# ishine/TargetDiarization

Measured on AMD Instinct MI355X. Metric: real-time factor (audio-sec/wall-sec) full infer() pipe, 16kHz mono, 1/2/4/8 GPU, higher is better.
Workload: dtype f32 (split-f16 x3: fp32-accurate products from three f16 MFMA passes, fp32 accumulate); 1 GPU; BASELINE configs[3]: 1800 s synthetic conversation (two alternating speakers, 20 % overlap) = 180 x 10 s windows: MossFormer2 (90 windows per launch) -> loudness swap -> ERes2NetV2 on every 10 s window of both streams + cosine vs a target embedding -> Paraformer (SANM encoder, CIF predictor, NAR decoder, argmax tokens + timestamps) on 30 s segments of both streams -> CT-Transformer punctuation of ; windows_per_launch=90

## Files before the change

### targetdiarization_amd/_lib.py

```python
from __future__ import annotations

import ctypes as C
import os

HERE = os.path.dirname(os.path.abspath(__file__))
LIB_PATH = os.path.join(HERE, "libtdx.so")


class TdxError(RuntimeError):
    pass


class Mf2Config(C.Structure):
    _fields_ = [("num_blocks", C.c_int32), ("channels", C.c_int32), ("kernel_size", C.c_int32),
                ("num_spks", C.c_int32), ("group_size", C.c_int32), ("reserved", C.c_int32 * 3)]


class MdxConfig(C.Structure):
    _fields_ = [("num_blocks", C.c_int32), ("l", C.c_int32), ("g", C.c_int32), ("k", C.c_int32), ("bn", C.c_int32),
                ("dim_f", C.c_int32), ("dim_t", C.c_int32), ("reserved", C.c_int32)]


class WhisperConfig(C.Structure):
    _fields_ = [("n_mels", C.c_int32), ("n_audio_ctx", C.c_int32), ("d_model", C.c_int32), ("enc_heads", C.c_int32),
# ... 179 lines not shown
                           "(hipcc --offload-arch=gfx950).  There is no CPU fallback.")
        import torch
        tl = os.path.join(os.path.dirname(torch.__file__), "lib", "libamdhip64.so")
        if os.path.exists(tl):
            C.CDLL(tl, mode=C.RTLD_GLOBAL)
        l = C.CDLL(LIB_PATH)
        for name, (res, args) in SIGNATURES.items():
            fn = getattr(l, name)
            fn.restype = res
            fn.argtypes = args
        _lib = l
    return _lib


_l = C.c_long


class GemmSeg(C.Structure):
    _fields_ = [("A", _vp), ("B", _vp), ("lda", _l), ("ldb", _l), ("strideA", _l), ("strideB", _l), ("strideA2", _l), ("strideB2", _l),
                ("K", _i), ("zdiv", _i), ("kchunk", _i), ("ktotal", _i)]


class H3Seg(C.Structure):
    _fields_ = [("A", _vp), ("B", _vp), ("sa", _vp), ("sb", _vp), ("lda", _l), ("ldb", _l),
                ("strideA", _l), ("strideB", _l), ("strideA2", _l), ("strideB2", _l),
                ("strideSA", _l), ("strideSB", _l), ("strideSA2", _l), ("strideSB2", _l),
                ("sa_mul", _i), ("sb_mul", _i), ("K", _i), ("zdiv", _i), ("kchunk", _i), ("ktotal", _i), ("segk", _i),
                ("strideSeg", _l), ("a_shift", _i), ("a_period", _i), ("a_zero", _vp)]


DIAG_SIGNATURES = {
    "tdx_diag_last_error": (C.c_char_p, []),
    "tdx_h3_gemm_ex": (_i, [_i] * 4 + [C.POINTER(H3Seg)] * 2 + [_i] * 12 + [_vp, _vp, _l, _l, _i, C.POINTER(_i), _vp]),
    "tdx_h3_plan": (_i, [_i] * 5 + [C.POINTER(_i)] * 2),
    "tdx_h3_tile_of_block": (_i, [C.POINTER(_i), _i, _i, _i] + [C.POINTER(_i)] * 3),
    "tdx_h3_split_rows_static": (_i, [_vp, _l, _vp, _l, _i, C.c_float, _vp]),
    "tdx_h3_split_rows_long": (_i, [_vp, _l, _vp, _vp, _l, _i, _vp]),
    "tdx_h3_split_kmajor_ex": (_i, [_vp, _l, _vp, _l, _i, C.c_float, _i, _vp, _vp, _i, _i, _vp]),
    "tdx_h3_split_rows": (_i, [_vp, _l, _vp, _vp, _l, _i, _vp]),
    "tdx_h3_split_kmajor": (_i, [_vp, _l, _vp, _l, _i, C.c_float, _vp]),
    "tdx_h3_gemm_x": (_i, [_i] + [_vp] * 5 + [_i] * 3 + [_vp]),
    "tdx_h3_gemm": (_i, [_vp] * 6 + [_i] * 3 + [_vp]),
    "tdx_h3_gemm_variant": (_i, [_vp] * 6 + [_i] * 4 + [_vp]),
    "tdx_linear_variant": (_i, [_vp, _vp, _i, _i, _i, _vp, _i, _vp]),
    "tdx_linear_epi": (_i, [_vp] * 5 + [_i] * 5 + [_vp]),
    "tdx_gemm_f32": (_i, [_i] * 3 + [C.POINTER(GemmSeg)] * 2 + [_i] * 5 + [_vp, _l, _l, _i, C.POINTER(_i), _vp]),
    "tdx_gemm_f32_conv": (_i, [_vp, _l, _vp] + [_i] * 11 + [_vp, _l, _i, C.POINTER(_i), _vp]),
    "tdx_attn_gate_planes_workspace_bytes": (_sz, [_i, _i, _i]),
    "tdx_attn_gate_planes": (_i, [_vp] * 7 + [_i] * 5 + [_vp] * 5 + [_sz, _vp]),
    "tdx_diag_dft_analysis": (_i, [_i, _i, _l, _l, _l, _i, _vp]),
    "tdx_diag_dft_synthesis": (_i, [_i, _i, _l, _l, _i, _vp]),
    "tdx_diag_loader_bind": (_i, [_vp, _sz] + [_i] * 9 + [_vp, _sz, C.POINTER(_i)]),
    "tdx_test_whisper_noise": (_i, [C.c_ulonglong, C.c_ulonglong, _i, _i, _i, _vp, _vp, _vp]),
    "tdx_fill_bench": (_i, [_i, _vp, _l, _i, _i, _vp, _vp]),
    "tdx_fill_bench2": (_i, [_i, _vp, _i, _i, _i, _vp, _vp]),
    "tdx_fill_bench3": (_i, [_vp, _l, _i, _l, _i, _i, _i, _vp, _vp]),
}
DIAG_PATH = os.path.join(HERE, "libtdx_diag.so")
_diag = None


def diag():
    global _diag
    if _diag is None:
        if not os.path.exists(DIAG_PATH):
            raise TdxError(f"{DIAG_PATH} not found: build it with `python -m targetdiarization_amd.build`")
# ... 152 lines not shown
```

### targetdiarization_amd/csrc/diag.hip

```cpp
#include <hip/hip_runtime.h>

#include <algorithm>
#include <climits>
#include <initializer_list>
#include <string>

#include "../../include/tdx.h"
#include "../../include/tdx_test.h"
#include "dft_basis.hpp"
#include "epilogues.hpp"
#include "mf2_attention.hpp"
#include "weight_pack.hpp"
#include "whisper_noise.hpp"

using namespace tdx;

namespace {
template <class Act>
int linear_epi(const float* a, const float* w, const float* bias, const float* res, float* out, int M, int Npad, int nreal, int K, hipStream_t st) {
    if (res && nreal < Npad) return linear_f32(a, K, w, M, Npad, K, EpiBiasResN<Act>{bias, res, out, Npad, nreal}, st);
    if (res) return linear_f32(a, K, w, M, Npad, K, EpiBiasRes<Act>{bias, res, out, Npad}, st);
    if (nreal < Npad) return linear_f32(a, K, w, M, Npad, K, EpiBiasActN<Act>{bias, out, Npad, nreal}, st);
    return linear_f32(a, K, w, M, Npad, K, EpiBiasAct<Act>{bias, out, Npad}, st);
}

struct EpiPlainN {
    float* out; long ld, strideZ; int nreal;
    __device__ EpiNone col(int, int) const { return EpiNone{}; }
    __device__ EpiNone row(int, int) const { return EpiNone{}; }
    __device__ void store(int z, int m, int n, float v, EpiNone, EpiNone) const {
        if (n < nreal) out[(long)z * strideZ + (long)m * ld + n] = v;
    }
};
struct EpiPlainPair {
    float* out; long ld, strideZ; int nreal, pair_off;
    __device__ EpiNone col(int, int) const { return EpiNone{}; }
    __device__ EpiNone row(int, int) const { return EpiNone{}; }
    __device__ void store2(int z, int m, int c, float v0, float v1, EpiNone, EpiNone) const {
        if (c < nreal) {
            float* o = out + (long)z * strideZ + (long)m * ld;
            o[c] = v0; o[pair_off + c] = v1;
        }
    }
// ... 292 lines not shown
            if (s && s->ldb < 4L * (pair_off + N)) return bad("need ldb >= 4 * (pair_off + N) bytes with a K-major B");
    H3Args g{};
    g.seg[0] = h3_seg_of(*seg0);
    if (seg1_or_null) g.seg[1] = h3_seg_of(*seg1_or_null);
    g.nseg = seg1_or_null ? 2 : 1; g.M = M; g.N = N; g.pair_off = pair_off;
    if (a_conv) {
        const int nt = taps_total ? taps_total : ntaps;
        if (!zero_row) return bad("A_CONV without zero_row");
        if (nt != 1 && nt != 9) return bad("need 1 or 9 taps in all");
        if (ntaps < 1 || taps_total < 0 || (taps_total && taps_total % ntaps)) return bad("need ntaps >= 1, taps_total % ntaps == 0");
        if (batches != (taps_total ? taps_total / ntaps : 1)) return bad("need batches == taps_total / ntaps (1 without taps_total)");
        if (cin < 64 || cin % 16) return bad("need cin >= 64, cin % 16 == 0");
        if (seg0->K != ntaps * cin) return bad("need K == ntaps * cin");
        if (seg0->lda < 4L * cin) return bad("need lda >= 4 * cin bytes");
        if (Hin < 1 || Win < 1 || Hout < 1 || Wout < 1 || stride < 1) return bad("need positive extents, stride >= 1");
        if ((long)Hout * Wout > 0x7fffffffL || M % (Hout * Wout)) return bad("need M == B * Hout * Wout");
        if ((long)(M / (Hout * Wout)) * Hin * Win > 0x7fffffffL) return bad("rows beyond int");
        g.cv_Hin = Hin; g.cv_Win = Win; g.cv_Hout = Hout; g.cv_Wout = Wout; g.cv_stride = stride; g.cv_ntaps = ntaps; g.cv_cin = cin;
        g.cv_taps_total = taps_total; g.zero_row = (const unsigned char*)zero_row;
    }
    hipStream_t st = (hipStream_t)stream;
    if (paired) {
        const EpiPlainPair e{out, ldo, strideO, nreal, pair_off};
        return b_kmajor ? run_gemm_h3<true, true, true, false>(g, batches, e, plan_or_null, st)
                        : run_gemm_h3<false, true, false, false>(g, batches, e, plan_or_null, st);
    }
    const EpiPlainN e{out, ldo, strideO, nreal};
    if (a_conv) return run_gemm_h3<false, false, false, true>(g, batches, e, plan_or_null, st);
    if (twoseg) return run_gemm_h3<false, false, true, false>(g, batches, e, plan_or_null, st);
    if (b_kmajor) return run_gemm_h3<true, false, false, false>(g, batches, e, plan_or_null, st);
    return run_gemm_h3<false, false, false, false>(g, batches, e, plan_or_null, st);
}

int tdx_h3_plan(int M, int N, int ktot, int batches, int paired, int* plan, int* grid) {
    if (!plan || !grid || M < 1 || N < 1 || ktot < 16 || batches < 1 || (paired && N % 128)) return tdx::fail(TDX_E_INVALID, "tdx_h3_plan: bad argument");
    H3Args g{};
    g.nseg = 1; g.seg[0].K = ktot; g.M = M; g.N = N;
    const dim3 gr = paired ? plan_gemm_h3<true, EpiPlainPair>(g, batches) : plan_gemm_h3<false, EpiPlainN>(g, batches);
    h3_plan_out(g, plan);
    grid[0] = (int)gr.x; grid[1] = (int)gr.y;
    return TDX_OK;
}
int tdx_h3_tile_of_block(const int* plan, int batches, int bx, int by, int* z, int* bm, int* bn) {
    if (!plan || !z || !bm || !bn || bx < 0 || by < 0 || batches < 1 || plan[2] < 1 || plan[4] < 1 || plan[5] < 1 || plan[3] < 0 ||
        (plan[0] == 0 && plan[1] < 1)) {
        tdx::fail(TDX_E_INVALID, "tdx_h3_tile_of_block: bad argument");
        return -1;
    }
    H3Args g{};
    g.map_mode = plan[0]; g.mp = plan[1]; g.gw = plan[2]; g.mc = plan[3]; g.tiles_m = plan[4]; g.tiles_n = plan[5]; g.batches = batches;
    *z = *bm = *bn = -1;
    return h3_tile_of_block(g, (unsigned)bx, (unsigned)by, *z, *bm, *bn) ? 1 : 0;
}

int tdx_h3_split_rows_static(const float* x, long ld, void* planes, long R, int K, float s, void* stream) {
    if (!x || !planes || R < 1 || K < 8 || K % 8 || ld < K || ld % 4 || !(s > 0.f) || !(s < 3e38f))
        return tdx::fail(TDX_E_INVALID, "tdx_h3_split_rows_static: need R >= 1, K % 8 == 0, ld >= K, ld % 4 == 0, 0 < s < inf");
    hipError_t r = tdx::launch_h3_split_rows_static(x, ld, planes, R, K, s, (hipStream_t)stream);
    return r == hipSuccess ? TDX_OK : tdx::fail_hip(r, __FILE__, __LINE__);
}
int tdx_h3_split_rows_long(const float* x, long ld, void* planes, float* scale, long R, int K, void* stream) {
    if (!x || !planes || !scale || R < 1 || K < 16 || K % 16 || ld < K || ld % 4)
        return tdx::fail(TDX_E_INVALID, "tdx_h3_split_rows_long: need R >= 1, K % 16 == 0, ld >= K, ld % 4 == 0");
    hipError_t r = tdx::launch_h3_split_rows_long(x, ld, planes, scale, R, K, (hipStream_t)stream);
    return r == hipSuccess ? TDX_OK : tdx::fail_hip(r, __FILE__, __LINE__);
}
// ... 188 lines not shown
```

### targetdiarization_amd/csrc/eres2net.hip

```cpp
#include <hip/hip_runtime.h>

#include <algorithm>
#include <cmath>
#include <string>
#include <vector>

#include "../../include/tdx.h"
#include "epilogues.hpp"
#include "weight_pack.hpp"
#include "weight_planes.hpp"

using namespace tdx;

namespace {

constexpr int NSTAGE = 4, SCALE = 4, EMB = 192;
const int kBlocks[NSTAGE] = {3, 4, 6, 3};
const int kPlanes[NSTAGE] = {64, 128, 256, 512};
const int kStride[NSTAGE] = {1, 2, 2, 2};

__global__ __launch_bounds__(256) void stem_kernel(const float* __restrict__ feat, const float* __restrict__ w9,
                                                    const float* __restrict__ bias, float* __restrict__ out, int F, long rows) {
    const long i = (long)blockIdx.x * 256 + threadIdx.x;
    if (i >= rows * 16) return;
    const long m = i >> 4;
    const int c = (int)(i & 15) * 4;
    const int w = (int)(m % F), h = (int)((m / F) % 80), b = (int)(m / ((long)F * 80));
    float4 acc = *reinterpret_cast<const float4*>(bias + c);
#pragma unroll
    for (int t = 0; t < 9; ++t) {
        const int ih = h + t / 3 - 1, iw = w + t % 3 - 1;
        if (ih >= 0 && ih < 80 && iw >= 0 && iw < F) {
            const float x = feat[((long)b * F + iw) * 80 + ih];
            const float4 k = *reinterpret_cast<const float4*>(w9 + t * 64 + c);
            acc.x = fmaf(k.x, x, acc.x); acc.y = fmaf(k.y, x, acc.y); acc.z = fmaf(k.z, x, acc.z); acc.w = fmaf(k.w, x, acc.w);
        }
    }
    acc.x = fmaxf(acc.x, 0.f); acc.y = fmaxf(acc.y, 0.f); acc.z = fmaxf(acc.z, 0.f); acc.w = fmaxf(acc.w, 0.f);
    *reinterpret_cast<float4*>(out + m * 64 + c) = acc;
}

// ... 392 lines not shown
}

struct ConvW : tdx::GemmW {
    const unsigned char* hp = nullptr; const float* hs = nullptr;
};
struct AffW { ConvW c0, c3; int C, inter, ipad; };
struct BlockW { ConvW conv1, convs[4], conv3, sc; bool has_sc; AffW aff[3]; int stride, cin, width, wpad, w4, cout; bool is_aff; };

template <class Epi>
int conv_gemm(const float* A, long lda, const float* dev, const ConvW& cw, int B, int Hin, int Win, int Hout, int Wout, int stride,
              Epi e, hipStream_t st) {
    const long M = (long)B * Hout * Wout;
    GemmArgs g = make_args((int)M, cw.Npad, make_seg(A, lda, dev + cw.w, (long)cw.taps * cw.cinp, cw.cinp));
    g.n_valid = up(cw.N, 32);
    g.cv_Hin = Hin; g.cv_Win = Win; g.cv_Hout = Hout; g.cv_Wout = Wout; g.cv_stride = stride; g.cv_ntaps = cw.taps; g.cv_cin = cw.cinp;
    if (launch_gemm<false, false, false, false, Epi, 0, true>(g, 1, e, st) != hipSuccess) return tdx::fail_hip(hipGetLastError(), __FILE__, __LINE__);
    return TDX_OK;
}

template <class Epi>
int conv_gemm_h3(const unsigned char* Ap, const float* inv_scale, const unsigned char* zero_row, const ConvW& cw, int B, int Hin, int Win,
                 int Hout, int Wout, int stride, Epi e, hipStream_t st) {
    const long M = (long)B * Hout * Wout;
    H3Args g{};
    g.seg[0] = h3_seg(Ap, inv_scale, 4L * cw.cinp, cw.hp, cw.hs, 4L * cw.taps * cw.cinp, cw.taps * cw.cinp);
    g.seg[0].sa_mul = 0;
    g.nseg = 1; g.M = (int)M; g.N = cw.Npad;
    g.cv_Hin = Hin; g.cv_Win = Win; g.cv_Hout = Hout; g.cv_Wout = Wout; g.cv_stride = stride; g.cv_ntaps = cw.taps; g.cv_cin = cw.cinp;
    g.zero_row = zero_row;
    if (launch_gemm_h3x<false, false, false, false, Epi, 0, true>(g, 1, e, st) != hipSuccess) return tdx::fail_hip(hipGetLastError(), __FILE__, __LINE__);
    return TDX_OK;
}

constexpr long DS_SPLIT_ROWS = 4096;
constexpr int DS_SPLIT = 3;
inline int conv_gemm_h3_tapsplit(const unsigned char* Ap, const float* inv_scale, const unsigned char* zero_row, const ConvW& cw, int B, int Hin, int Win,
                                 int Hout, int Wout, int stride, float* slab, const float* bias, float* out, hipStream_t st) {
    const long M = (long)B * Hout * Wout;
    H3Args g{};
    const int tpb = cw.taps / DS_SPLIT;
    g.seg[0] = h3_seg(Ap, inv_scale, 4L * cw.cinp, cw.hp, cw.hs, 4L * cw.taps * cw.cinp, tpb * cw.cinp);
    g.seg[0].sa_mul = 0;
    g.seg[0].strideB = 4L * tpb * cw.cinp;
    g.nseg = 1; g.M = (int)M; g.N = cw.Npad;
    g.cv_Hin = Hin; g.cv_Win = Win; g.cv_Hout = Hout; g.cv_Wout = Wout; g.cv_stride = stride; g.cv_ntaps = tpb; g.cv_cin = cw.cinp;
    g.cv_taps_total = cw.taps;
    g.zero_row = zero_row;
    if (launch_gemm_h3x<false, false, false, false, EpiStoreZ, 0, true>(g, DS_SPLIT, EpiStoreZ{slab, (long)cw.Npad, M * cw.Npad}, st) != hipSuccess)
        return tdx::fail_hip(hipGetLastError(), __FILE__, __LINE__);
    const long MN = M * cw.Npad;
    hipLaunchKernelGGL(slab_reduce_kernel, dim3((unsigned)((MN / 4 + 255) / 256)), dim3(256), 0, st, slab, DS_SPLIT, MN, cw.Npad, bias, out);
    LAUNCH_CHECK();
    return TDX_OK;
}

}

struct tdx_eres2net {
    int device = 0;
    tdx::DevBuf dev; std::vector<BlockW> blocks; size_t stem_w, stem_b, seg_w, seg_b; ConvW ds; AffW fuse34;
    tdx::DevBuf dev_planes;
    size_t consts = 0;
};

namespace {

// ... 85 lines not shown
        const int planes = kPlanes[s], width = planes * 24 / 64, cout = planes * 4;
        for (int i = 0; i < kBlocks[s] && ld.ok(); ++i) {
            const std::string p = "layer" + std::to_string(s + 1) + "." + std::to_string(i) + ".";
            BlockW b;
            b.stride = i == 0 ? kStride[s] : 1; b.cin = in_planes; b.width = width; b.wpad = up(width, 32); b.w4 = width * SCALE;
            b.cout = cout; b.is_aff = s >= 2;
            b.conv1 = fold(p + "conv1.weight", "", p + "bn1.", b.w4, in_planes, 1);
            for (int j = 0; j < SCALE; ++j) b.convs[j] = fold(p + "convs." + std::to_string(j) + ".weight", "", p + "bns." + std::to_string(j) + ".", width, width, 9);
            b.conv3 = fold(p + "conv3.weight", "", p + "bn3.", cout, b.w4, 1);
            b.has_sc = (b.stride != 1) || (in_planes != cout);
            if (b.has_sc) b.sc = fold(p + "shortcut.0.weight", "", p + "shortcut.1.", cout, in_planes, 1);
            if (b.is_aff) for (int j = 0; j < SCALE - 1; ++j) b.aff[j] = fold_aff(p + "fuse_models." + std::to_string(j) + ".", width);
            h->blocks.push_back(b);
            in_planes = cout;
        }
    }
    if (ld.ok()) {
        h->ds = fold("layer3_ds.weight", "", "", 2048, 1024, 9);
        h->fuse34 = fold_aff("fuse34.", 2048);
        h->seg_w = ld.push(ld.get("seg_1.weight", (size_t)EMB * 40960), (size_t)EMB * 40960);
        h->seg_b = ld.push(ld.get("seg_1.bias", EMB), EMB);
    }
    h->consts = ld.room(64 + 2048);
    ld.host[h->consts] = 1.0f / 1024.0f;
    ld.host[h->consts + 1] = 1.0f / 512.0f;
    h->device = device;
    TRY(ld.finish("tdx_eres2net_create", false, device, h->dev));
    {
        std::vector<ConvW*> jobs;
        size_t bi = 0;
        for (int s = 0; s < NSTAGE; ++s)
            for (int i = 0; i < kBlocks[s]; ++i, ++bi) {
                BlockW& b = h->blocks[bi];
                if (s < 1) { for (int j = 0; j < SCALE; ++j) jobs.push_back(&b.convs[j]); continue; }
                jobs.push_back(&b.conv1); if (b.has_sc) jobs.push_back(&b.sc);
                for (int j = 0; j < SCALE; ++j) jobs.push_back(&b.convs[j]);
                jobs.push_back(&b.conv3);
            }
        jobs.push_back(&h->ds);
        jobs.push_back(&h->fuse34.c0); jobs.push_back(&h->fuse34.c3);
        std::vector<tdx::PlaneJob> planes;
        for (ConvW* c : jobs) planes.push_back({h->dev + c->w, c->Npad, c->taps * c->cinp, &c->hp, &c->hs, tdx::launch_h3_split_rows_long});
        TRY(tdx::split_weight_planes(planes, device, h->dev_planes));
    }
    *out = h.release();
    return TDX_OK;
}

int tdx_eres2net_destroy(tdx_eres2net* h) {
    delete h;
    return TDX_OK;
}

namespace {
struct WsPlan { size_t P, keep3, o1, spin, tbuf, stats, hx, hcat, hin, slab, total; };
inline WsPlan ws_plan(const tdx_eres2net* h, int B, int F) {
    const Dims d = make_dims(F);
    WsPlan w{}; size_t mP = (size_t)B * 80 * F * 64, mo1 = 0, msp = 0, mt = 0, mhx = 0, mhc = 0, mhi = 0;
    int s = 0, cnt = 0;
    for (const BlockW& b : h->blocks) {
        const size_t rows = (size_t)B * d.H[s + 1] * d.W[s + 1];
        if (s >= 1) {
            const size_t rows_in = cnt == 0 ? (size_t)B * d.H[s] * d.W[s] : rows;
            mhx = std::max(mhx, rows_in * b.cin); mhc = std::max(mhc, rows * b.w4); mhi = std::max(mhi, rows * b.wpad);
        }
        mP = std::max(mP, rows * b.cout); mo1 = std::max(mo1, rows * b.w4); msp = std::max(msp, rows * b.wpad);
// ... 26 lines not shown
        const double pos = (double)d.H[s + 1] * d.W[s + 1];
        fl += 2.0 * pos * ((double)b.cin * b.w4 + 4.0 * 9 * b.width * b.width + (double)b.w4 * b.cout + (b.has_sc ? (double)b.cin * b.cout : 0.0));
        if (b.is_aff) fl += 3.0 * 2.0 * pos * (2.0 * b.width * (b.width / 4) + (double)(b.width / 4) * b.width);
        if (++cnt == kBlocks[s]) { cnt = 0; ++s; }
    }
    const double pos4 = (double)d.H[4] * d.W[4];
    fl += 2.0 * pos4 * (9.0 * 1024 * 2048 + 4096.0 * 512 + 512.0 * 2048) + 2.0 * 40960 * EMB;
    return fl * B;
}

int tdx_eres2net_forward(tdx_eres2net* h, const float* feat, int B, int F, float* emb, void* ws_, size_t ws_bytes, void* stream) {
    if (!h || !feat || !emb || !ws_ || B < 1) return tdx::fail(TDX_E_INVALID, "tdx_eres2net_forward: bad argument");
    if (F < 9) return tdx::fail(TDX_E_INVALID, "tdx_eres2net_forward: need >= 9 fbank frames (TSTP needs >= 2 pooled frames)");
    const WsPlan wp = ws_plan(h, B, F);
    if (ws_bytes < wp.total * sizeof(float)) return tdx::fail(TDX_E_WORKSPACE, "tdx_eres2net_forward: workspace too small");
    tdx::DeviceGuard guard(h->device);
    if (guard.err != hipSuccess) return tdx::fail_hip(guard.err, __FILE__, __LINE__);
    hipStream_t st = (hipStream_t)stream;
    const Dims d = make_dims(F);
    const size_t rows1 = (size_t)B * 80 * F;
    float* ws = (float*)ws_;
    float* P[3] = {ws, ws + wp.P, ws + 2 * wp.P};
    float* keep3 = ws + 3 * wp.P;
    float* o1 = keep3 + wp.keep3; float* cat = o1 + wp.o1;
    float* spin[2] = {cat + wp.o1, cat + wp.o1 + wp.spin};
    float* tbuf = spin[1] + wp.spin; float* stats = tbuf + wp.tbuf;
    unsigned char* hx = (unsigned char*)(stats + wp.stats);
    unsigned char* hcat = hx + wp.hx * sizeof(float);
    unsigned char* hin = hcat + wp.hcat * sizeof(float);
    float* slab = reinterpret_cast<float*>(hin + wp.hin * sizeof(float));
    const float* inv20 = h->dev + h->consts;
    const float* inv40 = h->dev + h->consts + 1;
    const unsigned char* zero_row = (const unsigned char*)(h->dev + h->consts + 64);

    hipLaunchKernelGGL(stem_kernel, dim3((unsigned)((rows1 * 16 + 255) / 256)), dim3(256), 0, st, feat, h->dev + h->stem_w, h->dev + h->stem_b, P[0], F, (long)rows1);
    LAUNCH_CHECK();
    const float* x = P[0];
    int cur = 0;
    int s = 0, cnt = 0;
    for (const BlockW& b : h->blocks) {
        const int Hin = (cnt == 0) ? d.H[s] : d.H[s + 1], Win = (cnt == 0) ? d.W[s] : d.W[s + 1];
        const int Ho = d.H[s + 1], Wo = d.W[s + 1];
        const long M = (long)B * Ho * Wo;
        const bool last_of_stage3 = (s == 2) && (cnt == kBlocks[2] - 1);
        const int iy = cur < 0 ? 0 : (cur + 1) % 3, ir = cur < 0 ? 1 : (cur + 2) % 3;
        float* y = last_of_stage3 ? keep3 : P[iy];
        float* res = P[ir];
        const bool x3 = b.conv1.hp != nullptr;
        const float* resid = x;
        if (x3) {
            int Hc = Hin, Wc = Win, sc_ = b.stride;
            if (b.stride == 2 && b.cin % 16 == 0) {
                const long R = (long)B * Ho * Wo;
                hipLaunchKernelGGL(split_rows_static_s2_kernel, dim3((unsigned)((R * (b.cin / 8) + 255) / 256)), dim3(256), 0, st,
                                   x, b.cin, hx, R, b.cin, Hin, Win, Ho, Wo, 1024.0f);
                LAUNCH_CHECK();
                Hc = Ho; Wc = Wo; sc_ = 1;
            } else if (tdx::launch_h3_split_rows_static(x, b.cin, hx, (long)B * Hin * Win, b.cin, 1024.0f, st) != hipSuccess)
                return tdx::fail_hip(hipGetLastError(), __FILE__, __LINE__);
            TRY(conv_gemm_h3(hx, inv20, zero_row, b.conv1, B, Hc, Wc, Ho, Wo, sc_, EpiBiasActN<ActRelu20>{h->dev + b.conv1.b, o1, b.w4, b.w4}, st));
            if (b.has_sc) {
                TRY(conv_gemm_h3(hx, inv20, zero_row, b.sc, B, Hc, Wc, Ho, Wo, sc_, EpiBiasActN<>{h->dev + b.sc.b, res, b.cout, b.cout}, st));
                resid = res;
            }
        } else {
            TRY(conv_gemm(x, b.cin, h->dev, b.conv1, B, Hin, Win, Ho, Wo, b.stride, EpiBiasActN<ActRelu20>{h->dev + b.conv1.b, o1, b.w4, b.w4}, st));
            if (b.has_sc) {
                TRY(conv_gemm(x, b.cin, h->dev, b.sc, B, Hin, Win, Ho, Wo, b.stride, EpiBiasActN<>{h->dev + b.sc.b, res, b.cout, b.cout}, st));
                resid = res;
            }
        }
        for (int j = 0; j < SCALE; ++j) {
            const float* in = j == 0 ? o1 : spin[j & 1];
            const long ldin = j == 0 ? b.w4 : b.wpad;
            const bool plain_next = (j + 1 < SCALE) && !b.is_aff;
            EpiChain e{h->dev + b.convs[j].b, cat, b.w4, j * b.width, b.width, b.wpad, o1, b.w4, (j + 1) * b.width,
                       plain_next ? spin[(j + 1) & 1] : nullptr};
            if (b.convs[j].hp && !b.is_aff && (b.width == 24 || b.width == 48)) {
                ChainX3Args ca{in, ldin, b.convs[j].hp, b.convs[j].hs, 9 * b.convs[j].cinp, b.convs[j].cinp, h->dev + b.convs[j].b, cat, b.w4, j * b.width,
                               o1, b.w4, (j + 1) * b.width, plain_next ? spin[(j + 1) & 1] : nullptr, b.wpad, Ho, Wo};
                if (b.width == 24) TRY((launch_chain_x3<24, 4>(ca, B, st)));
                else TRY((launch_chain_x3<48, 4>(ca, B, st)));
            } else if (x3) {
                if (tdx::launch_h3_split_rows_static(in, ldin, hin, M, b.wpad, 512.0f, st) != hipSuccess)
                    return tdx::fail_hip(hipGetLastError(), __FILE__, __LINE__);
                TRY(conv_gemm_h3(hin, inv40, zero_row, b.convs[j], B, Ho, Wo, Ho, Wo, 1, e, st));
            } else {
                TRY(conv_gemm(in, ldin, h->dev, b.convs[j], B, Ho, Wo, Ho, Wo, 1, e, st));
            }
            if (b.is_aff && j + 1 < SCALE)
                TRY(run_aff(h, b.aff[j], cat + j * b.width, b.w4, o1 + (j + 1) * b.width, b.w4, tbuf, spin[(j + 1) & 1], b.wpad, M, st));
        }
        if (x3) {
            if (tdx::launch_h3_split_rows_static(cat, b.w4, hcat, M, b.w4, 1024.0f, st) != hipSuccess)
                return tdx::fail_hip(hipGetLastError(), __FILE__, __LINE__);
            TRY(conv_gemm_h3(hcat, inv20, zero_row, b.conv3, B, Ho, Wo, Ho, Wo, 1, EpiBiasRes<ActRelu20>{h->dev + b.conv3.b, resid, y, b.cout}, st));
        } else {
            TRY(linear_f32(cat, b.w4, h->dev + b.conv3.w, (int)M, b.conv3.Npad, b.conv3.cinp, EpiBiasRes<ActRelu20>{h->dev + b.conv3.b, resid, y, b.cout}, st));
        }
        x = y;
        cur = last_of_stage3 ? -1 : iy;
        if (++cnt == kBlocks[s]) { cnt = 0; ++s; }
    }
    const int i_ds = (cur + 1) % 3, i_fu = (cur + 2) % 3;
    const long M4 = (long)B * d.H[4] * d.W[4];
    if (tdx::launch_h3_split_rows_static(keep3, 1024, hx, (long)B * d.H[3] * d.W[3], 1024, 1024.0f, st) != hipSuccess)
        return tdx::fail_hip(hipGetLastError(), __FILE__, __LINE__);
    if (wp.slab && h->ds.taps == 9 && h->ds.Npad == 2048)
        TRY(conv_gemm_h3_tapsplit(hx, inv20, zero_row, h->ds, B, d.H[3], d.W[3], d.H[4], d.W[4], 2, slab, nullptr, P[i_ds], st));
    else
        TRY(conv_gemm_h3(hx, inv20, zero_row, h->ds, B, d.H[3], d.W[3], d.H[4], d.W[4], 2, EpiBiasActN<>{nullptr, P[i_ds], 2048, 2048}, st));
    const char* aff34_env = getenv("TDX_ERES_AFF34_ROWS");
    const long aff34_min = aff34_env ? atol(aff34_env) : 8192;
    if (M4 >= aff34_min && 2 * M4 <= (long)B * 40960 && h->fuse34.c0.hp && h->fuse34.ipad == 512)
        TRY(run_aff34_x3(h, h->fuse34, x, P[i_ds], tbuf, P[i_fu], M4, hx, hcat, stats, hin, stats + M4, inv20, st));
    else
        TRY(run_aff(h, h->fuse34, x, 2048, P[i_ds], 2048, tbuf, P[i_fu], 2048, M4, st));
    hipLaunchKernelGGL(tstp_kernel, dim3(d.H[4], B), dim3(256), 0, st, P[i_fu], stats, d.W[4], 2048, d.H[4]);
    LAUNCH_CHECK();
    hipLaunchKernelGGL(seg_kernel, dim3(EMB, B), dim3(256), 0, st, stats, h->dev + h->seg_w, h->dev + h->seg_b, emb, 40960);
    LAUNCH_CHECK();
    return TDX_OK;
}

}
```

Baseline: 497.6 audio-s/s.

## Fuse fp32-to-f16 hi/lo split into 1x1 conv GEMM for early ERes2Net stages

Adds a new split-f16 GEMM kernel that reads fp32 activations directly, splits them into hi/lo f16 planes inside LDS, and feeds the three-pass MFMA pipeline. ERes2Net stage 0 and stage 1 conv1, shortcut and conv3 1x1 convolutions now use it, removing the separate split_rows pass and its extra global round trip. Stage 0 also gains weight-plane packing for conv1/conv3 so these layers leave the plain fp32 GEMM path. The fused kernel carries an extra raw-fp32 LDS staging buffer and in-kernel conversion work, and is controlled by an environment level that defaults on.

Measured after the change: 503.6 audio-s/s, median of 6. 1.2% higher.

```diff
diff --git a/targetdiarization_amd/_lib.py b/targetdiarization_amd/_lib.py
--- a/targetdiarization_amd/_lib.py
+++ b/targetdiarization_amd/_lib.py
@@ -235,6 +235,7 @@
 DIAG_SIGNATURES = {
     "tdx_diag_last_error": (C.c_char_p, []),
     "tdx_h3_gemm_ex": (_i, [_i] * 4 + [C.POINTER(H3Seg)] * 2 + [_i] * 12 + [_vp, _vp, _l, _l, _i, C.POINTER(_i), _vp]),
+    "tdx_h3_gemm_f32a": (_i, [_vp, _l, C.c_float, _vp, _vp, _vp] + [_i] * 8 + [_vp, _l, _i, _vp]),
     "tdx_h3_plan": (_i, [_i] * 5 + [C.POINTER(_i)] * 2),
     "tdx_h3_tile_of_block": (_i, [C.POINTER(_i), _i, _i, _i] + [C.POINTER(_i)] * 3),
     "tdx_h3_split_rows_static": (_i, [_vp, _l, _vp, _l, _i, C.c_float, _vp]),
diff --git a/targetdiarization_amd/csrc/diag.hip b/targetdiarization_amd/csrc/diag.hip
--- a/targetdiarization_amd/csrc/diag.hip
+++ b/targetdiarization_amd/csrc/diag.hip
@@ -9,6 +9,7 @@
 #include "../../include/tdx_test.h"
 #include "dft_basis.hpp"
 #include "epilogues.hpp"
+#include "gemm_h3f.hpp"
 #include "mf2_attention.hpp"
 #include "weight_pack.hpp"
 #include "whisper_noise.hpp"
@@ -367,6 +368,27 @@
     return run_gemm_h3<false, false, false, false>(g, batches, e, plan_or_null, st);
 }
 
+int tdx_h3_gemm_f32a(const float* a, long lda, float a_mul, const float* inv_dev, const void* pb, const float* sb, int M, int N, int K,
+                     int Hin, int Win, int Hout, int Wout, int stride, float* out, long ldo, int nreal, void* stream) {
+    const auto bad = [](const char* m) { return tdx::fail(TDX_E_INVALID, std::string("tdx_h3_gemm_f32a: ") + m); };
+    if (!a || !inv_dev || !pb || !sb || !out) return bad("null argument");
+    if (M < 1 || N < 1 || K < 16 || K % 16) return bad("need M >= 1, N >= 1, K >= 16, K % 16 == 0");
+    if (lda < K || lda % 4) return bad("need lda >= K floats, lda % 4 == 0 (16-byte loads)");
+    if (!(a_mul > 0.f) || !(a_mul < 3e38f)) return bad("need 0 < a_mul < inf");
+    if (nreal < 1 || nreal > N || ldo < 1) return bad("need 1 <= nreal <= N, ldo >= 1");
+    if (Hin < 1 || Win < 1 || Hout < 1 || Wout < 1 || stride < 1) return bad("need positive extents, stride >= 1");
+    if ((long)Hout * Wout > 0x7fffffffL || M % (Hout * Wout)) return bad("need M == B * Hout * Wout");
+    if ((long)(Hout - 1) * stride >= Hin || (long)(Wout - 1) * stride >= Win) return bad("an output pixel reads outside the image");
+    if ((long)(M / (Hout * Wout)) * Hin * Win > 0x7fffffffL) return bad("rows beyond int");
+    H3Args g{};
+    g.seg[0] = h3_seg(a, inv_dev, 4L * lda, pb, sb, 4L * K, K);
+    g.seg[0].sa_mul = 0;
+    g.nseg = 1; g.M = M; g.N = N;
+    g.cv_Hin = Hin; g.cv_Win = Win; g.cv_Hout = Hout; g.cv_Wout = Wout; g.cv_stride = stride; g.cv_ntaps = 1; g.cv_cin = K;
+    const hipError_t r = launch_gemm_h3f(g, a_mul, EpiPlainN{out, ldo, 0, nreal}, (hipStream_t)stream);
+    return r == hipSuccess ? TDX_OK : tdx::fail_hip(r, __FILE__, __LINE__);
+}
+
 int tdx_h3_plan(int M, int N, int ktot, int batches, int paired, int* plan, int* grid) {
     if (!plan || !grid || M < 1 || N < 1 || ktot < 16 || batches < 1 || (paired && N % 128)) return tdx::fail(TDX_E_INVALID, "tdx_h3_plan: bad argument");
     H3Args g{};
diff --git a/targetdiarization_amd/csrc/eres2net.hip b/targetdiarization_amd/csrc/eres2net.hip
--- a/targetdiarization_amd/csrc/eres2net.hip
+++ b/targetdiarization_amd/csrc/eres2net.hip
@@ -7,6 +7,7 @@
 
 #include "../../include/tdx.h"
 #include "epilogues.hpp"
+#include "gemm_h3f.hpp"
 #include "weight_pack.hpp"
 #include "weight_planes.hpp"
 
@@ -465,6 +466,20 @@
     return TDX_OK;
 }
 
+template <class Epi>
+int conv_gemm_h3f(const float* A, long lda, float a_mul, const float* inv_scale, const ConvW& cw, int B, int Hin, int Win, int Hout, int Wout,
+                  int stride, Epi e, hipStream_t st) {
+    const long M = (long)B * Hout * Wout;
+    H3Args g{};
+    g.seg[0] = h3_seg(A, inv_scale, 4L * lda, cw.hp, cw.hs, 4L * cw.cinp, cw.cinp);
+    g.seg[0].sa_mul = 0;
+    g.nseg = 1; g.M = (int)M; g.N = cw.Npad;
+    g.cv_Hin = Hin; g.cv_Win = Win; g.cv_Hout = Hout; g.cv_Wout = Wout; g.cv_stride = stride; g.cv_ntaps = 1; g.cv_cin = cw.cinp;
+    if (cw.taps != 1 || !cw.hp || lda < cw.cinp) return tdx::fail(TDX_E_INVALID, "conv_gemm_h3f: a 1x1 convolution with weight planes and lda >= cinp");
+    const hipError_t r = launch_gemm_h3f(g, a_mul, e, st);
+    return r == hipSuccess ? TDX_OK : tdx::fail_hip(r, __FILE__, __LINE__);
+}
+
 constexpr long DS_SPLIT_ROWS = 4096;
 constexpr int DS_SPLIT = 3;
 inline int conv_gemm_h3_tapsplit(const unsigned char* Ap, const float* inv_scale, const unsigned char* zero_row, const ConvW& cw, int B, int Hin, int Win,
@@ -616,6 +631,7 @@
         for (int s = 0; s < NSTAGE; ++s)
             for (int i = 0; i < kBlocks[s]; ++i, ++bi) {
                 BlockW& b = h->blocks[bi];
+                if (s < 1) { if (i > 0) jobs.push_back(&b.conv1); jobs.push_back(&b.conv3); }
                 if (s < 1) { for (int j = 0; j < SCALE; ++j) jobs.push_back(&b.convs[j]); continue; }
                 jobs.push_back(&b.conv1); if (b.has_sc) jobs.push_back(&b.sc);
                 for (int j = 0; j < SCALE; ++j) jobs.push_back(&b.convs[j]);
@@ -708,6 +724,8 @@
     const float* inv20 = h->dev + h->consts;
     const float* inv40 = h->dev + h->consts + 1;
     const unsigned char* zero_row = (const unsigned char*)(h->dev + h->consts + 64);
+    const char* f32a_env = getenv("TDX_ERES_F32A");
+    const int f32a_level = f32a_env ? atoi(f32a_env) : 2;
 
     hipLaunchKernelGGL(stem_kernel, dim3((unsigned)((rows1 * 16 + 255) / 256)), dim3(256), 0, st, feat, h->dev + h->stem_w, h->dev + h->stem_b, P[0], F, (long)rows1);
     LAUNCH_CHECK();
@@ -722,9 +740,17 @@
         const int iy = cur < 0 ? 0 : (cur + 1) % 3, ir = cur < 0 ? 1 : (cur + 2) % 3;
         float* y = last_of_stage3 ? keep3 : P[iy];
         float* res = P[ir];
-        const bool x3 = b.conv1.hp != nullptr;
+        const bool x3 = s >= 1;
+        const bool f32a = (s == 0 && f32a_level >= 2) || (s == 1 && f32a_level >= 1);
+        const bool f32a_in = f32a && !(s == 0 && cnt == 0);
         const float* resid = x;
-        if (x3) {
+        if (f32a_in) {
+            TRY(conv_gemm_h3f(x, b.cin, 1024.0f, inv20, b.conv1, B, Hin, Win, Ho, Wo, b.stride, EpiBiasActN<ActRelu20>{h->dev + b.conv1.b, o1, b.w4, b.w4}, st));
+            if (b.has_sc) {
+                TRY(conv_gemm_h3f(x, b.cin, 1024.0f, inv20, b.sc, B, Hin, Win, Ho, Wo, b.stride, EpiBiasActN<>{h->dev + b.sc.b, res, b.cout, b.cout}, st));
+                resid = res;
+            }
+        } else if (x3) {
             int Hc = Hin, Wc = Win, sc_ = b.stride;
             if (b.stride == 2 && b.cin % 16 == 0) {
                 const long R = (long)B * Ho * Wo;
@@ -767,7 +793,9 @@
             if (b.is_aff && j + 1 < SCALE)
                 TRY(run_aff(h, b.aff[j], cat + j * b.width, b.w4, o1 + (j + 1) * b.width, b.w4, tbuf, spin[(j + 1) & 1], b.wpad, M, st));
         }
-        if (x3) {
+        if (f32a) {
+            TRY(conv_gemm_h3f(cat, b.w4, 1024.0f, inv20, b.conv3, B, Ho, Wo, Ho, Wo, 1, EpiBiasRes<ActRelu20>{h->dev + b.conv3.b, resid, y, b.cout}, st));
+        } else if (x3) {
             if (tdx::launch_h3_split_rows_static(cat, b.w4, hcat, M, b.w4, 1024.0f, st) != hipSuccess)
                 return tdx::fail_hip(hipGetLastError(), __FILE__, __LINE__);
             TRY(conv_gemm_h3(hcat, inv20, zero_row, b.conv3, B, Ho, Wo, Ho, Wo, 1, EpiBiasRes<ActRelu20>{h->dev + b.conv3.b, resid, y, b.cout}, st));
diff --git a/targetdiarization_amd/csrc/gemm_h3f.hpp b/targetdiarization_amd/csrc/gemm_h3f.hpp
--- /dev/null
+++ b/targetdiarization_amd/csrc/gemm_h3f.hpp
@@ -0,0 +1,276 @@
+#pragma once
+#include "gemm_h3.hpp"
+
+namespace tdx {
+
+constexpr int H3F_B = 0;
+constexpr int H3F_AI = 4 * H3_OPER;
+constexpr int H3F_RAW = H3F_AI + 2 * H3_OPER;
+constexpr int H3F_NRAW = 3;
+constexpr int H3F_LDS = H3F_RAW + H3F_NRAW * H3_OPER;
+
+template <int OFF>
+__device__ __forceinline__ void h3f_raw_read(f32x4& v, unsigned a) {
+    asm volatile("ds_read_b128 %0, %1 offset:%2" : "=v"(v) : "v"(a), "n"(OFF) : "memory");
+}
+__device__ __forceinline__ void h3f_raw_fence(f32x4 (&v)[4]) {
+    asm volatile("s_waitcnt lgkmcnt(0)" : "+v"(v[0]), "+v"(v[1]), "+v"(v[2]), "+v"(v[3]) :: "memory");
+}
+
+template <class Epi>
+__global__ __launch_bounds__(H3_THREADS, 2) void gemm_h3f_kernel(H3Args g, float a_mul, Epi epi) {
+    using RowT = decltype(epi.row(0, 0));
+    static_assert(std::is_empty<RowT>::value, "fp32-A form: functors without a row() value");
+    extern __shared__ __attribute__((aligned(1024))) unsigned char lds[];
+    const int tid = threadIdx.x;
+    const int lane = tid & 63, wave = tid >> 6;
+    const int l31 = lane & 31, h = lane >> 5;
+    const int wm = wave >> 2, wn = wave & 3;
+
+    int bm, bn;
+    {
+        const int x = blockIdx.x & 7, i = blockIdx.x >> 3;
+        const int tile = x * g.mp + i;
+        if (tile >= g.tiles_m * g.tiles_n) return;
+        bm = tile / g.tiles_n; bn = tile - bm * g.tiles_n;
+    }
+    constexpr int z = 0;
+    const int m0 = bm * H3_BM, n0 = bn * H3_BN;
+
+    f32x16 acc[4][2];
+#pragma unroll
+    for (int i = 0; i < 4; ++i)
+#pragma unroll
+        for (int j = 0; j < 2; ++j)
+#pragma unroll
+            for (int r = 0; r < 16; ++r) acc[i][j][r] = 0.f;
+
+    const bool stB = wave >= 4;
+    H3Frag f;
+    const int a0row = (wm * 128 + l31) * H3_ROWB;
+    {
+        const int fl = (l31 >> 2) & 3;
+        f.a0 = H3F_AI + a0row;
+        f.apl[0] = ((2 * h) ^ fl) << 4; f.apl[1] = ((2 * h + 1) ^ fl) << 4;
+#pragma unroll
+        for (int tm = 0; tm < 4; ++tm) f.at[tm] = 0;
+        f.b0 = (wn * 32 + l31) * H3_ROWB;
+        f.bpl[0] = f.apl[0]; f.bpl[1] = f.apl[1];
+    }
+    auto bstage = [&](int u) -> unsigned char* { return lds + H3F_B + (u & 3) * H3_OPER; };
+    auto frag_of = [&](int u) { H3Frag fu = f; fu.a0 = H3F_AI + ((u & 1) - (u & 3)) * H3_OPER + a0row; return fu; };
+    const bool full_n = n0 + 128 < g.N;
+    const bool wave_on = m0 + wm * 128 < g.M;
+
+    const H3Seg& sg = g.seg[0];
+    const int nkt = sg.K / H3_BK;
+    f16x8 ah[4], al[4], bh[2], bl[2];
+    auto first_frags = [&]() {
+#pragma unroll
+        for (int tn = 0; tn < 2; ++tn) {
+            bh[tn] = h3_frag<false>(h3_addr_b<false>(lds, f, tn, 0));
+            bl[tn] = h3_frag<false>(h3_addr_b<false>(lds, f, tn, 1));
+        }
+#pragma unroll
+        for (int tm = 0; tm < 4; ++tm) {
+            ah[tm] = h3_frag<false>(h3_addr_a<false>(lds, f, tm, 0));
+            al[tm] = h3_frag<false>(h3_addr_a<false>(lds, f, tm, 1));
+        }
+    };
+    const unsigned char* const nogp[4] = {lds, lds, lds, lds};
+    auto wait_keep = [&](int n) { if (n >= 2) H3_WAIT_VM(8); else if (n == 1) H3_WAIT_VM(4); else H3_WAIT_VM(0); };
+
+    if (stB) {
+        const int sdst = (wave & 3) * 4096;
+        const unsigned char* gp[4];
+#pragma unroll
+        for (int j = 0; j < 4; ++j) {
+            const int r = (wave & 3) * 64 + (lane >> 2) + 16 * j;
+            const int n = min(n0 + r, g.N - 1);
+            gp[j] = sg.B + (long)n * sg.ldb + (((lane & 3) ^ ((r >> 2) & 3)) << 4);
+        }
+#pragma unroll
+        for (int p = 0; p < 4; ++p)
+            if (p < nkt) {
+#pragma unroll
+                for (int j = 0; j < 4; ++j) h3_glds16(gp[j] + p * H3_ROWB, bstage(p) + sdst + j * 1024);
+            }
+        if (nkt >= 4) H3_WAIT_VM(12); else wait_keep(nkt - 1);
+        H3_BARRIER();
+        first_frags();
+        auto run = [&](auto fulln) {
+            constexpr bool FN = decltype(fulln)::value;
+            int t = 0;
+            for (; t + 4 < nkt; ++t) {
+                H3_WAIT_VM(8);
+                H3_BARRIER();
+                if (wave_on)
+                    h3_stage<false, false, FN, true, true, 1>(acc, ah, al, bh, bl, bstage(t + 1), frag_of(t + 1), gp, (long)(t + 4) * H3_ROWB,
+                                                              bstage(t + 4) + sdst);
+                else
+                    h3_stage_dma_only<true>(gp, (long)(t + 4) * H3_ROWB, bstage(t + 4) + sdst);
+            }
+            for (; t + 1 < nkt; ++t) {
+                wait_keep(nkt - 2 - t);
+                H3_BARRIER();
+                if (wave_on) h3_stage<false, false, FN, true, false, 1>(acc, ah, al, bh, bl, bstage(t + 1), frag_of(t + 1), nogp, 0, lds);
+            }
+            if (wave_on) h3_stage<false, false, FN, false, false, 1>(acc, ah, al, bh, bl, lds, f, nogp, 0, lds);
+        };
+        if (full_n) run(std::true_type{}); else run(std::false_type{});
+    } else {
+        const unsigned char* ar[4];
+        {
+            const int hw = g.cv_Hout * g.cv_Wout;
+#pragma unroll
+            for (int j = 0; j < 4; ++j) {
+                const int r = wave * 64 + 16 * j + (lane >> 2);
+                const int m = min(m0 + r, g.M - 1);
+                const int b_ = m / hw, r_ = m - b_ * hw;
+                const int h_ = r_ / g.cv_Wout, w_ = r_ - h_ * g.cv_Wout;
+                const long pix = (long)b_ * g.cv_Hin * g.cv_Win + (long)(h_ * g.cv_stride) * g.cv_Win + w_ * g.cv_stride;
+                ar[j] = sg.A + pix * sg.lda + (lane & 3) * 16;
+            }
+        }
+        const int q = lane & 3, r0 = wave * 64 + (lane >> 2);
+        const int ad0 = r0 * H3_ROWB + (((2 * (q >> 1)) ^ ((r0 >> 2) & 3)) << 4) + (q & 1) * 8;
+        const int rawoff = H3F_RAW + wave * 4096;
+        const unsigned rawrd = h3_lds_addr(lds) + rawoff + lane * 16;
+        auto dma = [&](int u, int slot) {
+#pragma unroll
+            for (int j = 0; j < 4; ++j) h3_glds16(ar[j] + (long)u * (H3_BK * 4), lds + rawoff + slot * H3_OPER + j * 1024);
+        };
+        auto advance = [&](int u, int slot) {
+            wait_keep(min(u + 2, nkt - 1) - u);
+            f32x4 v[4];
+            const unsigned ra = rawrd + slot * H3_OPER;
+            h3f_raw_read<0>(v[0], ra); h3f_raw_read<1024>(v[1], ra); h3f_raw_read<2048>(v[2], ra); h3f_raw_read<3072>(v[3], ra);
+            h3f_raw_fence(v);
+            if (u + 3 < nkt) dma(u + 3, slot);
+            unsigned char* img = lds + H3F_AI + (u & 1) * H3_OPER + ad0;
+#pragma unroll
+            for (int j = 0; j < 4; ++j) {
+                f16x4 hi, lo;
+#pragma unroll
+                for (int i = 0; i < 4; ++i) {
+                    const float xs = v[j][i] * a_mul;
+                    const _Float16 t = (_Float16)xs;
+                    hi[i] = t;
+                    lo[i] = (_Float16)(xs - (float)t);
+                }
+                *reinterpret_cast<f16x4*>(img + j * 1024) = hi;
+                *reinterpret_cast<f16x4*>((img + j * 1024) + ((ad0 & 16) ? -16 : 16)) = lo;
+            }
+        };
+#pragma unroll
+        for (int p = 0; p < H3F_NRAW; ++p)
+            if (p < nkt) dma(p, p);
+        advance(0, 0);
+        if (1 < nkt) advance(1, 1);
+        H3_BARRIER();
+        first_frags();
+        auto run = [&](auto fulln) {
+            constexpr bool FN = decltype(fulln)::value;
+            int slot = 2;
+            for (int t = 0; t + 1 < nkt; ++t) {
+                H3_BARRIER();
+                if (t + 2 < nkt) advance(t + 2, slot);
+                slot = slot == H3F_NRAW - 1 ? 0 : slot + 1;
+                if (wave_on) h3_stage<false, false, FN, true, false, 0>(acc, ah, al, bh, bl, bstage(t + 1), frag_of(t + 1), nogp, 0, lds);
+            }
+            if (wave_on) h3_stage<false, false, FN, false, false, 0>(acc, ah, al, bh, bl, lds, f, nogp, 0, lds);
+        };
+        if (full_n) run(std::true_type{}); else run(std::false_type{});
+    }
+
+    const float sr = sg.sa[0];
+    const float* sb = sg.sb;
+    const int sbm = sg.sb_mul;
+    const int lrow0 = wm * 128 + 4 * h, lcol0 = wn * 32 + l31;
+    auto epilogue = [&](auto tag) {
+        constexpr bool CHECK = decltype(tag)::value;
+        int lrow = lrow0, lcol = lcol0;
+        asm volatile("" : "+v"(lrow), "+v"(lcol));
+        auto rowm = [&](int lr) { return CHECK ? min(m0 + lr, g.M - 1) : m0 + lr; };
+        int nn[2];
+        decltype(epi.col(0, 0)) cc[2];
+        float sc[2];
+#pragma unroll
+        for (int tn = 0; tn < 2; ++tn) {
+            nn[tn] = n0 + tn * 128 + lcol;
+            const int nc = min(nn[tn], g.N - 1);
+            cc[tn] = epi.col(z, nc);
+            sc[tn] = sb[(long)nc * sbm];
+        }
+        touch(cc[0]); touch(cc[1]); touch(sc[0]); touch(sc[1]);
+        if constexpr (epi_has_aux<Epi>::value) {
+            constexpr int AH = H3_AUX_AHEAD;
+            decltype(epi.aux(0, 0, 0, RowT{})) ax[AH + 1][8];
+            auto fetch = [&](int i, int set) {
+                const int tn = i >> 3, tm = (i >> 1) & 3, half = i & 1;
+                int lb = lrow + tm * 32;
+                asm volatile("" : "+v"(lb));
+#pragma unroll
+                for (int r8 = 0; r8 < 8; ++r8) {
+                    const int r = half * 8 + r8;
+                    const int lr = lb + (r & 3) + 8 * (r >> 2);
+                    ax[set][r8] = epi.aux(z, rowm(lr), min(nn[tn], g.N - 1), RowT{});
+                }
+            };
+#pragma unroll
+            for (int i = 0; i < AH; ++i) fetch(i, i % (AH + 1));
+#pragma unroll
+            for (int i = 0; i < 16; ++i) {
+                __builtin_amdgcn_sched_barrier(0);
+                if (i + AH < 16) fetch(i + AH, (i + AH) % (AH + 1));
+                const int tn = i >> 3, tm = (i >> 1) & 3, half = i & 1;
+                int lb = lrow + tm * 32;
+                asm volatile("" : "+v"(lb));
+#pragma unroll
+                for (int r8 = 0; r8 < 8; ++r8) touch(ax[i % (AH + 1)][r8]);
+                if (nn[tn] < g.N) {
+#pragma unroll
+                    for (int r8 = 0; r8 < 8; ++r8) {
+                        const int r = half * 8 + r8;
+                        const int lr = lb + (r & 3) + 8 * (r >> 2);
+                        if (!CHECK || m0 + lr < g.M)
+                            epi.store(z, m0 + lr, nn[tn], acc[tm][tn][r] * (sr * sc[tn]), RowT{}, cc[tn], ax[i % (AH + 1)][r8]);
+                    }
+                }
+            }
+        } else {
+#pragma unroll
+            for (int tn = 0; tn < 2; ++tn) {
+                if (nn[tn] >= g.N) continue;
+#pragma unroll
+                for (int tm = 0; tm < 4; ++tm) {
+#pragma unroll
+                    for (int r = 0; r < 16; ++r) {
+                        const int lr = lrow + tm * 32 + (r & 3) + 8 * (r >> 2);
+                        if (!CHECK || m0 + lr < g.M) epi.store(z, m0 + lr, nn[tn], acc[tm][tn][r] * (sr * sc[tn]), RowT{}, cc[tn]);
+                    }
+                }
+            }
+        }
+    };
+    if (m0 + 256 <= g.M) epilogue(std::false_type{}); else epilogue(std::true_type{});
+}
+
+template <class Epi>
+inline hipError_t launch_gemm_h3f(H3Args g, float a_mul, Epi epi, hipStream_t st) {
+    static const hipError_t attr_rc = hipFuncSetAttribute(reinterpret_cast<const void*>(&gemm_h3f_kernel<Epi>), hipFuncAttributeMaxDynamicSharedMemorySize, H3F_LDS);
+    (void)attr_rc;
+    const H3Seg& sg = g.seg[0];
+    if (g.nseg != 1 || g.M < 1 || g.N < 1 || sg.K < 16 || sg.K % 16 || sg.sa_mul != 0 || !sg.A || !sg.B || !sg.sa || !sg.sb) return hipErrorInvalidValue;
+    if (sg.lda < 4L * sg.K || sg.lda % 16 || sg.ldb < 4L * sg.K || sg.ldb % 16 || !(a_mul > 0.f)) return hipErrorInvalidValue;
+    if (g.cv_Hin < 1 || g.cv_Win < 1 || g.cv_Hout < 1 || g.cv_Wout < 1 || g.cv_stride < 1 || g.M % (g.cv_Hout * g.cv_Wout)) return hipErrorInvalidValue;
+    if ((long)(g.cv_Hout - 1) * g.cv_stride >= g.cv_Hin || (long)(g.cv_Wout - 1) * g.cv_stride >= g.cv_Win) return hipErrorInvalidValue;
+    g.tiles_m = (g.M + H3_BM - 1) / H3_BM;
+    g.tiles_n = (g.N + H3_BN - 1) / H3_BN;
+    g.batches = 1;
+    g.mp = (g.tiles_m * g.tiles_n + 7) / 8;
+    hipLaunchKernelGGL((gemm_h3f_kernel<Epi>), dim3(8 * g.mp), dim3(H3_THREADS), H3F_LDS, st, g, a_mul, epi);
+    return hipGetLastError();
+}
+
+}
```
